# marlam/wurblpt

Measured on AMD Instinct MI355X. Metric: Msamples/s, higher is better.
Workload: dtype f32; 1 GPU; cornell_1024x1024_1024spp_ggx_glass; width=1024, height=1024, spp=1024, triangles=36, bvh_nodes=71, parallelism=1 launch

## Files before the change

wurblpt_amd/csrc/wpt_capi.hip:

```cpp
#include <hip/hip_runtime.h>

#include <algorithm>
#include <atomic>
#include <cassert>
#include <cfloat>
#include <cmath>
#include <cstring>
#include <memory>
#include <string>
#include <vector>

#include "../../include/wurblpt_hip.h"
#include "wpt_pathtrace.inc.h"
#include "wpt_kernel_table.h"
#include "wpt_launch_plan.h"
#include "wpt_scene_layout.h"
#include "wpt_bypass.h"
#include "wpt_wavefront.inc.h"
#include "wpt_postproc.h"
#include "wpt_lightmix.h"
#include "wpt_denoise_launch.h"
#include "wpt_progress.h"
#include "wpt_progress_state.h"

using namespace wptd;
using namespace wptk;

namespace {

__global__ void wpt_selftest_kernel(int op, int n, const float* a, const float* b, float* out)
{
    int i = blockIdx.x * blockDim.x + threadIdx.x;
    if (i >= n)
        return;
    float x = a[i], y = b[i], r;
    switch (op) {
    case 0: r = wptm::sinf_(x); break;
    case 1: r = wptm::cosf_(x); break;
    case 2: r = wptm::expf_(x); break;
    case 3: r = wptm::powf_(x, y); break;
    case 4: r = wptm::asinf_(x); break;
    case 5: r = wptm::atan2f_(x, y); break;
    case 6: r = x / y; break;
    case 7: r = __builtin_sqrtf(x); break;
    case 8: r = x * y + x; break;
    case 10: r = wptm::acosf_(x); break;
    case 11: r = wptm::atan2f_(x, 1.0f); break;
    case 12: r = (float)(2.0 * wptm::asin_d((double)x)); break;
    case 13:
    case 14: {
        float s, c;
        wptm::sincosf_(x, &s, &c);
        r = op == 13 ? s : c;
        break;
    }
    case 15:
    case 16: {
        f2 u;
        u.x = x;
        u.y = y;
        const f2 d = inUnitDisk(u);
        r = op == 15 ? d.x : d.y;
        break;
    }
    default: r = 1.0f / x; break;
    }
    out[i] = r;
}

__global__ void wpt_selftest_aabb_kernel(int n, const float* boxes, const float* rays, int32_t* out)
// ... 133 lines not shown
    wptpp::V3 rgb;
    rgb.x = in[3 * i];
    rgb.y = in[3 * i + 1];
    rgb.z = in[3 * i + 2];
    if (op == 0) {
        uint8_t* o = static_cast<uint8_t*>(out) + 3 * i;
        o[0] = wptpp::toSrgbByte<DevicePow>(rgb.x);
        o[1] = wptpp::toSrgbByte<DevicePow>(rgb.y);
        o[2] = wptpp::toSrgbByte<DevicePow>(rgb.z);
    } else if (op == 3) {
        const float y = wptpp::luminance(rgb);
        if (y > 0.0f)
            atomicMax(maxBits, __float_as_uint(y));
    } else {
        const wptpp::V3 r = op == 1 ? wptpp::uniformRationalQuantization(rgb, a, b) : wptpp::scaleLuminance(rgb, a, b);
        float* o = static_cast<float*>(out) + 3 * i;
        o[0] = r.x;
        o[1] = r.y;
        o[2] = r.z;
    }
}


thread_local std::string g_error;

wpt_status fail(wpt_status s, const std::string& msg)
{
    g_error = msg;
    return s;
}

#define HIP_TRY(expr)                                                                              \
    do {                                                                                           \
        hipError_t e_ = (expr);                                                                    \
        if (e_ != hipSuccess)                                                                      \
            return fail(WPT_ERR_HIP, std::string(#expr) + ": " + hipGetErrorString(e_));           \
    } while (0)
#define WPT_TRY(expr)                                                                              \
    do {                                                                                           \
        const wpt_status s_ = (expr);                                                              \
        if (s_ != WPT_OK)                                                                          \
            return s_;                                                                             \
    } while (0)

}

struct wpt_scene {
    int device;
    SceneView view;
    uint32_t features;
    uint32_t nodeCount, triCount;
    uint32_t foldedLinks;
    uint32_t* ldsLinks = nullptr;
    uint32_t bypassedNodes = 0;
    uint32_t animationCount;
    std::vector<void*> allocations;
    int cuCount;
    std::vector<float> envM, envMcs;
    std::vector<int32_t> envMs;
};

namespace {

uint32_t g_threadsPerGroup = WG;
uint32_t g_variant = 0;
uint32_t g_leaveEighths = 0;
uint32_t g_heavyMin = 0;
uint32_t g_leafBias = 0;
std::atomic<uint32_t> g_lastPasses{1};
std::atomic<const char*> g_kernelName{nullptr};
std::atomic<const char*> g_kernelForm{""};
uint32_t g_topNodes = 65536;
unsigned long long* g_schedStats = nullptr;
uint32_t g_wfMode = 0;
wptk::WfConfig g_wfConfig = { 0, 0, 0, 1, 0, 0, 0, 0, 0 };
uint32_t g_walk = 0;
uint32_t g_bypassMode = wptb::MODE_MODEL;
uint32_t g_slices = 0;
constexpr int SLICE_STATS_DEVICES = 64;
std::atomic<unsigned long long*> g_sliceStats[SLICE_STATS_DEVICES];
std::atomic<unsigned long long*> g_lastSliceStats{nullptr};
static_assert(wptk::PLAN_WG == uint32_t(WG) && wptk::PLAN_SLICE_SLOT_MAX == wptk::SLICE_SLOT_MASK && wptk::SLICE_UNITS_TARGET <= wptk::SLICE_UNITS_MAX
        && wptk::PLAN_FRAME == wptk::SENSOR_FRAME && wptk::PLAN_VIEWS == wptk::SENSOR_VIEWS && wptk::PLAN_ADAPTIVE == wptk::SENSOR_ADAPTIVE
        && wptk::PLAN_SENSORS == wptk::SENSOR_COUNT, "wpt_launch_plan.h restates the kernels' constants and the sensors");
static_assert(wptl::NODE_CHILD == NODE_CHILD && wptl::NODE_INDEX_MASK == NODE_INDEX_MASK && wptl::PRIM_SPHERE == PRIM_SPHERE && wptl::WIDE_STACK == WIDE_STACK
        && wptl::WIDE_NONE == WIDE_NONE && wptl::LDS_SCENE_MAX_BYTES == LDS_SCENE_MAX_BYTES, "wpt_scene_layout.h restates the kernels' node words and limits");

void recordLaunch(const char* name, const char* form, uint32_t passes, unsigned long long* sliceStats)
{
    g_kernelName.store(name, std::memory_order_relaxed);
    g_kernelForm.store(form, std::memory_order_relaxed);
    g_lastPasses.store(passes, std::memory_order_relaxed);
    g_lastSliceStats.store(sliceStats, std::memory_order_relaxed);
}

const char* kernelForm(bool rotated, uint32_t units = 0)
{
    static const std::vector<std::string> forms = [] {
        std::vector<std::string> f;
        for (int r = 0; r < 2; r++)
            for (uint32_t u = 0; u <= wptk::SLICE_UNITS_MAX; u++)
                f.push_back(std::string(r ? "rotated corners" : "") + (u > 1 ? ", sliced x" + std::to_string(u) : std::string()));
        return f;
    }();
    return forms[(rotated ? wptk::SLICE_UNITS_MAX + 1 : 0) + (units <= wptk::SLICE_UNITS_MAX ? units : 0)].c_str();
}

wpt_status lookupKernel(uint32_t features, bool count, bool ldsScene, bool wide, const wptk::KernelEntry** entry)
{
    *entry = wptk::findKernel(features, count, ldsScene, wide);
    if (!*entry)
        return fail(WPT_ERR_UNSUPPORTED, "the library has no kernel wpt_pathtrace<F = " + std::to_string(features) + ", COUNT = " + std::to_string(count)
                + ", LDSSCENE = " + std::to_string(ldsScene) + ", WIDE = " + std::to_string(wide) + ">");
    return WPT_OK;
}

unsigned long long* sliceStatsOfCurrentDevice()
{
    int dev = 0;
    if (hipGetDevice(&dev) != hipSuccess || dev < 0 || dev >= SLICE_STATS_DEVICES)
        return nullptr;
    unsigned long long* p = g_sliceStats[dev].load(std::memory_order_acquire);
    if (!p) {
        if (hipMalloc(reinterpret_cast<void**>(&p), 2 * sizeof(unsigned long long)) != hipSuccess) {
            (void)hipGetLastError();
            return nullptr;
        }
        unsigned long long* expected = nullptr;
        if (!g_sliceStats[dev].compare_exchange_strong(expected, p, std::memory_order_acq_rel)) {
            (void)hipFree(p);
            p = expected;
        }
    }
    return p;
}

template<typename T> wpt_status uploadArray(wpt_scene* s, const T* src, size_t count, const T** dst)
{
    *dst = nullptr;
    size_t bytes = count * sizeof(T);
    void* p = nullptr;
    hipError_t e = hipMalloc(&p, bytes > 0 ? bytes : 16);
    if (e != hipSuccess)
        return fail(e == hipErrorOutOfMemory ? WPT_ERR_OUT_OF_MEMORY : WPT_ERR_HIP, std::string("hipMalloc: ") + hipGetErrorString(e));
    s->allocations.push_back(p);
    if (bytes > 0)
        HIP_TRY(hipMemcpy(p, src, bytes, hipMemcpyHostToDevice));
    *dst = static_cast<const T*>(p);
    return WPT_OK;
}

wpt_status uploadQuads(wpt_scene* s, const std::vector<wptl::Quad>& quads, const float4** dst)
{
    static_assert(sizeof(wptl::Quad) == sizeof(float4), "the layout's quadwords are the device's");
    return uploadArray(s, reinterpret_cast<const float4*>(quads.data()), quads.size(), dst);
}

wpt_status layoutStatus(const wptl::Status& st)
// ... 142 lines not shown
{
    if (!device)
        return fail(WPT_ERR_INVALID_ARGUMENT, "device is NULL");
    HIP_TRY(hipGetDevice(device));
    return WPT_OK;
}

wpt_status wpt_scene_upload(const wpt_scene_desc* desc, wpt_scene** out_scene)
{
    if (!out_scene)
        return fail(WPT_ERR_INVALID_ARGUMENT, "out_scene is NULL");
    *out_scene = nullptr;
    WPT_TRY(validate(desc));
    if (wpt_device_count() <= 0)
        return fail(WPT_ERR_NO_DEVICE, "no HIP device is available; the path tracer has no CPU fallback");
    const uint32_t walk = g_walk, topNodes = g_topNodes;
    std::unique_ptr<wpt_scene, SceneFree> owner(new wpt_scene);
    wpt_scene* s = owner.get();
    SceneView& view = s->view;
    HIP_TRY(hipGetDevice(&s->device));
    s->features = sceneFeatures(desc);
    s->nodeCount = desc->node_count;
    s->triCount = desc->tri_count;
    memset(&view, 0, sizeof(view));
    const std::vector<uint32_t> triNew = wptl::triangleOrder(desc, (walk & WPT_WALK_TRIANGLES_AS_GIVEN) != 0);
    const bool fitsLds = size_t(desc->node_count) * 32 + size_t(desc->tri_count) * 48 <= LDS_SCENE_MAX_BYTES;
    std::vector<uint32_t> ldsNodes;
    {
        wptl::DeviceNodes nodes;
        WPT_TRY(layoutStatus(wptl::deviceNodes(desc, triNew, topNodes, &nodes)));
        view.nodeCount = desc->node_count;
        view.boxesMayBeNan = nodes.boxesMayBeNan;
        WPT_TRY(uploadQuads(s, nodes.quads, &view.nodes));
        s->foldedLinks = 0;
        if (fitsLds) {
            s->foldedLinks = wptl::countFoldedLinks(reinterpret_cast<const uint32_t*>(nodes.quads.data()), desc->node_count, nullptr);
            ldsNodes.resize(size_t(desc->node_count) * 8);
            memcpy(ldsNodes.data(), nodes.quads.data(), ldsNodes.size() * 4);
        }
    }
    if (walk & WPT_WALK_WIDE) {
        const std::vector<wptl::Quad> wide = wptl::wideNodes(desc, triNew);
        if (!wide.empty())
            WPT_TRY(uploadQuads(s, wide, &view.wideNodes));
    }
    {
        const std::vector<wpt_tri_geom> g = wptl::permuted(desc->tri_geom, triNew);
        WPT_TRY(uploadArray(s, reinterpret_cast<const float4*>(g.data()), size_t(desc->tri_count) * 3, &view.triGeom));
        if (fitsLds) {
            const wptb::Plan plan = wptb::plan(ldsNodes.data(), desc->node_count, g.data(), desc->tri_count, g_bypassMode);
            std::vector<uint32_t> words(plan.plain);
            words.insert(words.end(), plan.folded.begin(), plan.folded.end());
            words.insert(words.end(), plan.bypass.begin(), plan.bypass.end());
            const uint32_t* onDevice = nullptr;
            WPT_TRY(uploadArray(s, words.data(), words.size(), &onDevice));
            s->ldsLinks = const_cast<uint32_t*>(onDevice);
            s->bypassedNodes = plan.outCount;
        }
    }
    {
        const std::vector<wpt_tri_attr> a = wptl::permuted(desc->tri_attr, triNew);
        WPT_TRY(uploadArray(s, reinterpret_cast<const float4*>(a.data()), size_t(desc->tri_count) * 6, &view.triAttr));
    }
    WPT_TRY(uploadArray(s, desc->instances, desc->instance_count, &view.instances));
    WPT_TRY(uploadArray(s, desc->materials, desc->material_count, &view.materials));
    view.materialCount = desc->material_count;
    {
        size_t texelCount = 0;
        const std::vector<wpt_texture> devTex = wptl::texelOffsets(desc, &texelCount);
        WPT_TRY(uploadArray(s, devTex.data(), devTex.size(), &view.textures));
        WPT_TRY(decodeTexels(s, desc, devTex, texelCount));
    }
    {
        const std::vector<wpt_hotspot> h = wptl::remappedHotspots(desc, triNew);
        WPT_TRY(uploadArray(s, h.data(), h.size(), &view.hotspots));
    }
    WPT_TRY(uploadArray(s, desc->spheres, desc->sphere_count, &view.spheres));
    WPT_TRY(uploadArray(s, desc->rgl_brdfs, desc->rgl_count, &view.rglBrdfs));
    {
        const wptl::RglPool rgl = wptl::rglPool(desc);
        WPT_TRY(uploadArray(s, rgl.pool.data(), rgl.pool.size(), &view.rglData));
        WPT_TRY(uploadArray(s, rgl.rgbl.data(), rgl.rgbl.size(), &view.rglRgbl));
    }
    WPT_TRY(uploadArray(s, desc->animations, desc->animation_count, &view.animations));
    WPT_TRY(uploadArray(s, desc->keyframes, desc->keyframe_count, &view.keyframes));
    s->animationCount = desc->animation_count;
    view.sphereCount = desc->sphere_count;
    for (int k = 0; k < 6; k++)
        view.envCube[k] = desc->envmap.cube_tex[k];
    {
        hipDeviceProp_t prop;
        s->cuCount = hipGetDeviceProperties(&prop, s->device) == hipSuccess ? prop.multiProcessorCount : 256;
    }
    view.triCount = desc->tri_count;
    view.hotspotCount = desc->hotspot_count;
    view.invHotspotCount = desc->hotspot_count ? 1.0f / float(desc->hotspot_count) : 0.0f;
    if (desc->hotspot_count > 0)
        WPT_TRY(hotspotFaces(s));
    view.envType = desc->envmap.type;
    view.envCompat = desc->envmap.compat;
    view.envTex = desc->envmap.tex;
    view.envN = 0;
    view.envLog2N = -1;
    if (desc->envmap.type != WPT_ENV_NONE && desc->envmap.N > 0) {
        const int N = desc->envmap.N;
        const size_t bins = size_t(N) * N;
// ... 181 lines not shown
    first.carry = second.carry = carry;
    first.cost = cost;
    run(first);
    orderByCost(first, order, work, run.stream, second);
    run(second);
    return true;
}

bool runAdaptiveOrder(const wptk::KernelArgs& args, const SingleKernel& run, StreamScratch& scratch)
{
    uint32_t *cost, *order, *work;
    if (!(cost = scratch.get<uint32_t>(args.blockSize)) || !(order = scratch.get<uint32_t>(args.blockSize)) || !(work = scratch.get<uint32_t>(ORDER_WORK_WORDS)))
        return false;
    wptk::KernelArgs measure = args, ordered = args;
    measure.cost = cost - args.blockStart;
    wptk::launchAdaptiveCost(measure, run.stream);
    orderByCost(measure, order, work, run.stream, ordered);
    run(ordered);
    return true;
}

unsigned long long* runSliced(const wptk::KernelArgs& args, const SingleKernel& runTwin, const wptk::LaunchPlan& plan, StreamScratch& scratch)
{
    unsigned long long* stats = sliceStatsOfCurrentDevice();
    float4* carry;
    uint32_t* words;
    if (!stats || !(carry = scratch.get<float4>(size_t(args.blockSize) * 2)) || !(words = scratch.get<uint32_t>(args.blockSize)))
        return nullptr;
    if (hipMemsetAsync(words, 0, size_t(args.blockSize) * sizeof(uint32_t), runTwin.stream) != hipSuccess
            || hipMemsetAsync(stats, 0, 2 * sizeof(unsigned long long), runTwin.stream) != hipSuccess) {
        (void)hipGetLastError();
        return nullptr;
    }
    wptk::KernelArgs inSlices = args;
    inSlices.slices = { words, carry, stats, plan.rows, plan.units, (g_slices & WPT_SLICES_DECLINE_ODD) ? 1u : 0u };
    runTwin(inSlices);
    return stats;
}

hipError_t runSingleKernel(const wpt_scene* scene, wptk::KernelArgs& args, const wptk::KernelChoice& choice, const wptk::KernelEntry* kernel,
        const wptk::KernelEntry* slicedTwin, const wptk::LaunchPlan& plan, hipStream_t stream)
{
    StreamScratch scratch(stream);
    args.pool = plan.pooled ? scratch.get<uint32_t>(1) : nullptr;
    args.materialsInLds = choice.materialsInLds;
    if (choice.ldsScene) {
        if (!scene->ldsLinks)
            return hipErrorInvalidValue;
        const size_t words = 2 * size_t(scene->nodeCount) + 4;
        const bool fold = (choice.materialsInLds & wptk::LDS_FOLD) != 0;
        const bool bypass = fold && !(g_walk & WPT_WALK_NO_BYPASS) && !args.sv.boxesMayBeNan;
        args.sv.spheres = reinterpret_cast<const wpt_sphere*>(scene->ldsLinks + (fold ? words : 0));
        args.sv.wideNodes = reinterpret_cast<const float4*>(scene->ldsLinks + (bypass ? 2 * words : fold ? words : 0));
    }
    const SingleKernel run = { kernel, dim3((args.blockSize + WG - 1) / WG), choice.sceneLdsBytes, stream };
    bool done = false;
    unsigned long long* sliceStats = nullptr;
    if (args.pool && plan.strategy == wptk::TWO_PASSES)
        done = runTwoPasses(args, run, scratch);
    else if (args.pool && plan.strategy == wptk::ADAPTIVE_ORDER)
        done = runAdaptiveOrder(args, run, scratch);
    else if (args.pool && plan.strategy == wptk::SLICED)
        done = (sliceStats = runSliced(args, SingleKernel{ slicedTwin, run.grid, run.sceneLdsBytes, stream }, plan, scratch)) != nullptr;
    if (!done)
        run(args);
    recordLaunch(kernel->name, kernelForm(choice.rotated, sliceStats ? plan.units : 0), done ? plan.passes : 1u, sliceStats);
    return hipGetLastError();
}

wpt_status renderLaunch(const LaunchRequest& rq)
{
    const bool planes = rq.sensor == wptk::SENSOR_TRANSIENT || rq.sensor == wptk::SENSOR_TOF, views = rq.sensor == wptk::SENSOR_VIEWS;
    if (!rq.scene || !rq.camera || !rq.params || !(rq.frame || planes))
        return fail(WPT_ERR_INVALID_ARGUMENT, "NULL argument");
    const uint32_t cameraCount = views ? rq.views.viewCount : 1u;
    const wpt_status checked = checkFrameBlock(rq.width, rq.height, &rq.samplesSqrt, rq.blockStart, rq.bandStride ? 0u : rq.blockSize, cameraCount);
    if (checked != WPT_OK || rq.blockSize == 0)
        return checked;
    KernelArgs args = {};
    uint32_t need = 0;
    const bool count = rq.counters != nullptr;
    WPT_TRY(launchSetUp(rq.scene, rq.camera, cameraCount, views, rq.params, rq.width, rq.height, rq.samplesSqrt, rq.blockStart,
            rq.blockSize, rq.bandPixels, rq.bandFirst, rq.bandStride, count, args, need));
    args.frame = rq.frame;
    args.counters = rq.counters;
    args.schedStats = g_schedStats;
    if (views)
        args.views = rq.views;
    else if (rq.sensor == wptk::SENSOR_ADAPTIVE)
        args.adaptive = rq.adaptive;
    else if (planes)
        args.bins = rq.bins;
    args.rowStop = rq.samplesSqrt;
    const wptk::KernelChoice choice = wptk::selectKernel({ need, rq.sensor, count, rq.scene->nodeCount, rq.scene->triCount,
            uint32_t(rq.scene->view.materialCount), rq.scene->view.wideNodes != nullptr, g_variant, g_walk });
    const wptk::KernelEntry *kernel = nullptr, *slicedTwin = nullptr;
    wpt_status found = lookupKernel(choice.features, choice.count, choice.ldsScene, choice.wide, &kernel);
    if (found == WPT_OK && choice.sceneInLds && rq.sensor == wptk::SENSOR_FRAME && !count)
        found = lookupKernel(choice.features | FEAT_SLICED, choice.count, choice.ldsScene, choice.wide, &slicedTwin);
    if (found != WPT_OK)
        return found;
    const bool rgl = (need & FEAT_RGL) != 0;
    hipStream_t stream = static_cast<hipStream_t>(rq.stream);
    const wptk::LaunchPlan plan = wptk::planLaunch({ rq.sensor, count, rgl, (need & FEAT_ANIM) != 0, choice.sceneInLds, rq.blockSize, rq.samplesSqrt,
            uint32_t(rq.scene->cuCount), g_variant, g_wfMode, g_slices });
    if (plan.wavefront) {
        uint32_t launches = 0;
        const hipError_t e = wptk::renderWavefront(args, rgl ? wptk::wfFullRgl() : (choice.basic ? wptk::wfBasic() : wptk::wfFull()), g_wfConfig, stream, &launches);
        if (e == hipSuccess) {
            recordLaunch("wf_trace + wf_shade", "", launches, nullptr);
            return WPT_OK;
        }
        if (!plan.wavefrontFallBack || e != hipErrorOutOfMemory)
            return fail(e == hipErrorOutOfMemory ? WPT_ERR_OUT_OF_MEMORY : WPT_ERR_HIP, std::string("wavefront render: ") + hipGetErrorString(e));
        (void)hipGetLastError();
    }
    HIP_TRY(runSingleKernel(rq.scene, args, choice, kernel, slicedTwin, plan, stream));
    return WPT_OK;
}
// ... 1362 lines not shown
```

wurblpt_amd/csrc/wpt_device.h:

```cpp
#ifndef WPT_DEVICE_H
#define WPT_DEVICE_H

#include <hip/hip_runtime.h>
#include <stdint.h>

#include "../../include/wurblpt_hip.h"
#include "wpt_math.h"
#include "wpt_triangle.h"
#include "wpt_anim.h"
#include "wpt_rgl.h"

namespace wptd {

#define WPT_CALL static inline __device__ __attribute__((noinline))


WPT_D float dot(f2 a, f2 b) { float d = 0.0f; d += a.x * b.x; d += a.y * b.y; return d; }
WPT_D float dot(f3 a, f3 b) { float d = 0.0f; d += a.x * b.x; d += a.y * b.y; d += a.z * b.z; return d; }
WPT_D f3 normalize(f3 v) { return divs(v, __builtin_sqrtf(dot(v, v))); }
WPT_D f3 cross(f3 v, f3 w) { return mk3(v.y * w.z - v.z * w.y, v.z * w.x - v.x * w.z, v.x * w.y - v.y * w.x); }
WPT_D f3 reflect(f3 i, f3 n) { return sub(i, scl(2.0f * dot(n, i), n)); }
WPT_D f3 refract(f3 i, f3 n, float eta)
{
    const float d = dot(n, i);
// ... 386 lines not shown
    wptanim::applyTrs(T, sp.center, r.center);
    r.radius = sp.radius * m;
    return r;
}

#ifdef WPT_SPHERE_HIT_INLINE
#define WPT_SPHERE_HIT WPT_D
#else
#define WPT_SPHERE_HIT static __device__ __attribute__((noinline))
#endif
template<uint32_t F = 0> WPT_SPHERE_HIT Hit finishSphereHit(SphereScene sv, Candidate c, f3 org, f3 dir, float time = 0.0f)
{
    wpt_sphere sp = sv.spheres[c.prim & ~PRIM_SPHERE];
    if ((F & FEAT_ANIM) && sp.animation >= 0) {
        const wpt_animation a = sv.animations[sp.animation];
        sp = sphereMoved(sp, wptanim::at<DeviceAnimMath>(sv.keyframes + a.first_keyframe, a.keyframe_count, time));
    }
    Hit h;
    h.a = c.a;
    h.prim = c.prim;
    h.material = sp.material;
    h.p = add(org, scl(c.a, dir));
    f3 n = normalize(sub(h.p, ld3(sp.center)));
    const f3 rn = quatRotate(sp.rotation, n);
    const float alpha = wptm::atan2f_(rn.x, rn.z);
    const float beta = wptm::asinf_(clampr(rn.y, -1.0f, +1.0f));
    h.tc.x = 0.5f * k_inv_pi * (alpha + k_pi);
    h.tc.y = k_inv_pi * (beta + 0.5f * k_pi);
    f3 t = mk3(wptm::cosf_(alpha), 0.0f, -wptm::sinf_(alpha));
    if (__builtin_fabsf(dot(rn, t)) >= k_cosOrthoAngleTolerance)
        t = mk3(0.0f, 0.0f, 0.0f);
    h.backside = false;
    if (dot(n, neg(dir)) < 0.0f) {
        h.backside = true;
        n = neg(n);
    }
    h.n = n;
    h.t = t;
    return h;
}

struct TriGeomFromScene {
    const float4* triGeom;
    WPT_D float4 operator()(uint32_t i) const { return triGeom[i]; }
};
template<uint32_t F = 0, class Tri4 = TriGeomFromScene>
WPT_D Hit finishHit(const SceneView& sv, const Candidate& c, f3 org, f3 dir, float time, Tri4 tri4)
{
    if ((F & FEAT_SPHERES) && (c.prim & PRIM_SPHERE))
        return finishSphereHit<F>(sphereScene(sv), c, org, dir, time);
    Hit h;
    h.a = c.a;
    h.prim = c.prim;
    const float4 g0 = tri4(3 * c.prim + 0);
    const float4 g1 = tri4(3 * c.prim + 1);
    const float4 g2 = tri4(3 * c.prim + 2);
    const uint32_t instance = __float_as_uint(g0.w);
    h.material = __float_as_uint(g1.w);
    const uint32_t flags = __float_as_uint(g2.w);
    const bool backfacing = c.invDet < 0.0f;
    const float bx = c.invDet * c.U, by = c.invDet * c.V, bz = c.invDet * c.W;
    h.p = add(org, scl(c.a, dir));
    const float4* at = sv.triAttr + 6 * (size_t)c.prim;
    const float4 a0 = at[0], a1 = at[1], a2 = at[2], a3 = at[3], a4 = at[4], a5 = at[5];
    const f3 n0 = mk3(a0.x, a0.y, a0.z), n1 = mk3(a0.w, a1.x, a1.y), n2 = mk3(a1.z, a1.w, a2.x);
    f3 nrm = add(add(scl(bx, n0), scl(by, n1)), scl(bz, n2));
    const bool transform = (flags & WPT_TRI_TRANSFORM) != 0;
    const float* N = sv.instances[instance].N;
    if (transform)
        nrm = mat3mul(N, nrm);
    float animationN[9];
    const bool animate = (F & FEAT_ANIM) && (flags & WPT_TRI_ANIMATE);
    if (animate) {
        const wptanim::Trs T = animationAt(sv, sv.instances[instance].animation, time);
        wptanim::toMat3(T.q, animationN);
        nrm = mat3mul(animationN, nrm);
    }
    nrm = normalize(nrm);
    if (backfacing)
        nrm = neg(nrm);
    h.n = nrm;
    h.tc.x = 0.0f;
    h.tc.y = 0.0f;
    if (flags & WPT_TRI_HAVE_TEXCOORDS) {
        h.tc.x = bx * a2.y + by * a2.w + bz * a3.y;
        h.tc.y = bx * a2.z + by * a3.x + bz * a3.z;
    }
    f3 tan = mk3(0.0f, 0.0f, 0.0f);
    if (flags & WPT_TRI_HAVE_TANGENTS) {
        const f3 t0 = mk3(a3.w, a4.x, a4.y), t1 = mk3(a4.z, a4.w, a5.x), t2 = mk3(a5.y, a5.z, a5.w);
        tan = add(add(scl(bx, t0), scl(by, t1)), scl(bz, t2));
        if (dot(tan, tan) > 0.0f) {
            if (transform)
                tan = mat3mul(N, tan);
            if (animate)
                tan = mat3mul(animationN, tan);
            tan = normalize(sub(tan, scl(dot(nrm, tan), nrm)));
        }
    }
    h.t = tan;
    h.backside = backfacing;
    return h;
}
template<uint32_t F = 0>
WPT_D Hit finishHit(const SceneView& sv, const Candidate& c, f3 org, f3 dir, float time = 0.0f)
{
    TriGeomFromScene fromScene;
    fromScene.triGeom = sv.triGeom;
    return finishHit<F>(sv, c, org, dir, time, fromScene);
}

WPT_D float srgbToRgb(float x)
// ... 799 lines not shown
```

wurblpt_amd/csrc/wpt_pathtrace.inc.h:

```cpp
#ifndef WPT_PATHTRACE_INC_H
#define WPT_PATHTRACE_INC_H

#include <hip/hip_runtime.h>

#include "../../include/wurblpt_hip.h"
#include "wpt_blocks.h"

namespace wptk {

using namespace wptd;

constexpr int WG = 256;
constexpr uint32_t NODE_CHILD = 0xc0000000u;
constexpr uint32_t NODE_INDEX_MASK = 0x3fffffffu;
constexpr uint32_t TABLE_BYTES = WPT_MATH_TABLE_WORDS * 8;
constexpr uint32_t COLD_BYTES = TABLE_BYTES + SLOT_COUNT * WG * 16;
constexpr uint32_t LDS_SCENE_MAX_BYTES = 20 * 1024;
constexpr uint32_t LDS_BYTES_PER_WORKGROUP_AT_FOUR = 160 * 1024 / 4;
constexpr uint32_t LDS_MATERIALS = 1u;
constexpr uint32_t LDS_FOLD = 2u;
static_assert(sizeof(wpt_material) % 16 == 0 && alignof(wpt_material) <= 16, "wpt_material must be a whole number of quadwords");
struct ViewsView {
    const wpt_camera* cams;
    uint32_t viewPixels;
    uint32_t viewCount;
};
struct AdaptiveView {
    const uint16_t* samplesSqrt;
    float* moments;
};
struct SlicesView {
    uint32_t* words;
    float4* carry;
    unsigned long long* stats;
    uint32_t rows, units;
    uint32_t declineOdd;
};
constexpr uint32_t SLICE_UNITS_MAX = 15;
constexpr uint32_t SLICE_SLOT_BITS = 28;
constexpr uint32_t SLICE_SLOT_MASK = (1u << SLICE_SLOT_BITS) - 1u;
struct KernelArgs {
    SceneView sv;
    wpt_camera cam;
    wpt_params par;
    uint32_t width, height, samplesSqrt;
    float invWidth, invHeight, invSamplesSqrt, invSamples;
    uint32_t blockStart, blockSize;
    uint32_t tiled;
    uint32_t bandPixels, bandFirst, bandStride;
    uint32_t leaveEighths;
    uint32_t heavyMin;
    uint32_t leafBias;
    uint32_t waitBelow;
    uint32_t fuse;
    uint32_t shadowWalksEnd;
    float* frame;
    uint32_t* pool;
    uint32_t rowStop;
    float4* carry;
    uint32_t* cost;
    const uint32_t* order;
    const uint32_t* orderCount;
    uint32_t cuCount;
    uint32_t materialsInLds;
    wpt_counters* counters;
    unsigned long long* schedStats;
    union {
        BinsView bins;
        ViewsView views;
        AdaptiveView adaptive;
        SlicesView slices;
    };
};
// ... 5 lines not shown
    bool inBlock = gid < args.blockSize;
    if (args.tiled) {
        const uint32_t tilesPerRow = args.width >> 3;
        const uint32_t tile = gid >> 6, lane = gid & 63u;
        const uint32_t tx = tile % tilesPerRow;
        uint32_t ty = tile / tilesPerRow;
        if (args.bandStride) {
            const uint32_t tileRowsPerBand = args.bandPixels / (args.width << 3);
            ty = (args.bandFirst + (ty / tileRowsPerBand) * args.bandStride) * tileRowsPerBand + ty % tileRowsPerBand;
        }
        pixel = args.blockStart + ((ty << 3) + (lane >> 3)) * args.width + (tx << 3) + (lane & 7u);
    } else if (args.bandStride) {
        pixel = (args.bandFirst + (gid / args.bandPixels) * args.bandStride) * args.bandPixels + gid % args.bandPixels;
    } else {
        pixel = args.blockStart + gid;
    }
    if (args.bandStride && pixel >= args.width * args.height)
        inBlock = false;
    if (!inBlock)
        pixel = args.blockStart;
    return inBlock;
}

enum { S_NODE = 0, S_LEAF = 1, S_SHADE = 2, S_NEEEND = 3, S_NEW = 4, S_DONE = 5, S_START = 6  };

constexpr uint32_t WIDE_STACK = 96;
constexpr uint32_t WIDE_NONE = 0xffffffffu;
constexpr int RAY_WALK_BINARY = 0x80;

WPT_D uint2 exactLinks(const SceneView& sv, uint32_t n)
{
    return *reinterpret_cast<const uint2*>(reinterpret_cast<const char*>(sv.spheres) + (n << 3));
}

template<uint32_t F, bool COUNT, bool LDSSCENE, int OCC, bool WIDE = false>
__global__ __launch_bounds__(WG, OCC) void wpt_pathtrace(const KernelArgs args)
{
    static_assert(!WIDE || (!LDSSCENE && !COUNT), "the wide walk: product kernels that fetch the scene from HBM (counting launches walk like the reference)");
    static_assert(!LDSSCENE || !(F & FEAT_SPHERES), "the LDS copy of the tree tells leaves (complemented word) from inner nodes by the sign bit: triangle leaves only");
    static_assert(!((F & FEAT_VIEWS) && (F & FEAT_TRANSIENT)), "a batch of views has no transient film (they share KernelArgs' union)");
    static_assert(!((F & FEAT_ADAPTIVE) && (F & (FEAT_VIEWS | FEAT_TRANSIENT))), "adaptive sampling has no views and no transient film (they share KernelArgs' union)");
    static_assert(!((F & FEAT_ADAPTIVE) && COUNT), "adaptive sampling has no counting build");
    static_assert(!((F & FEAT_TOF) && ((F & (FEAT_VIEWS | FEAT_TRANSIENT | FEAT_ADAPTIVE)) || COUNT)), "the time-of-flight sensor: one view, no other film, no counting build");
    static_assert(!((F & FEAT_SLICED) && ((F & (FEAT_VIEWS | FEAT_TRANSIENT | FEAT_ADAPTIVE | FEAT_TOF)) || COUNT)), "pixels in slices: plain product launches (they share KernelArgs' union)");
    static_assert(!LDSSCENE || (!WIDE && !(F & FEAT_SPHERES)), "the kernels with the scene in LDS carry their link words in SceneView::wideNodes and ::spheres (wpt_device.h): they may read neither as what it is named");
    constexpr bool VIEWS = (F & FEAT_VIEWS) != 0;
    constexpr bool ADAPTIVE = (F & FEAT_ADAPTIVE) != 0;
    constexpr bool SLICED = (F & FEAT_SLICED) != 0;
    constexpr bool ROTATED = (F & FEAT_ROTATED) != 0;
    static_assert(!ROTATED || (LDSSCENE && !(F & FEAT_ANIM)), "rotated copies of the corners: scenes at rest in LDS");
    constexpr bool PREFETCH = !LDSSCENE && !WIDE;
    constexpr int STEPS = LDSSCENE ? 3 : 1;
    constexpr int NEE_IN_WALK = LDSSCENE ? 0 : 4;
    extern __shared__ float4 lds[];
    float4* const ldsCold = lds + TABLE_BYTES / 16;
    float4* const ldsScene = ldsCold + SLOT_COUNT * WG;
#if defined(WPT_MATH_TABLES_IN_LDS) && defined(__HIP_DEVICE_COMPILE__)
    wptm::tables_to_lds(threadIdx.x);
#endif

    SceneView svInLds = args.sv;
    const SceneView& sv = LDSSCENE ? static_cast<const SceneView&>(svInLds) : args.sv;
    const wpt_params& par = args.par;
    const uint32_t nodeCount = sv.nodeCount;

    if (LDSSCENE) {
        const uint32_t n4 = 2 * nodeCount, t4 = 3 * sv.triCount;
        for (uint32_t i = threadIdx.x; i < n4; i += WG) {
            float4 q = sv.nodes[i];
            if (i & 1) {
                const uint2 links = reinterpret_cast<const uint2*>(sv.wideNodes)[i >> 1];
                q.z = __uint_as_float(links.x);
                q.w = __uint_as_float(links.y);
            }
            ldsScene[i] = q;
        }
        if (threadIdx.x < 2)
            ldsScene[n4 + threadIdx.x] = threadIdx.x == 0 ? make_float4(0.0f, 0.0f, 0.0f, 0.0f)
                    : make_float4(0.0f, 0.0f, __uint_as_float(nodeCount), __uint_as_float(nodeCount));
        for (uint32_t i = threadIdx.x; i < t4; i += WG)
            ldsScene[n4 + 2 + i] = sv.triGeom[i];
        if (ROTATED) {
            for (uint32_t i = threadIdx.x; i < t4; i += WG) {
                const float4 g = sv.triGeom[i];
                ldsScene[n4 + 2 + t4 + i] = make_float4(g.y, g.z, g.x, g.w);
                ldsScene[n4 + 2 + 2 * t4 + i] = make_float4(g.z, g.x, g.y, g.w);
            }
        }
        const uint32_t c4 = ROTATED ? 3 * t4 : t4;
        if (args.materialsInLds & LDS_MATERIALS) {
            const uint32_t m4 = sv.materialCount * (uint32_t)(sizeof(wpt_material) / 16);
            const float4* from = reinterpret_cast<const float4*>(sv.materials);
            for (uint32_t i = threadIdx.x; i < m4; i += WG)
                ldsScene[n4 + 2 + c4 + i] = from[i];
            svInLds.materials = reinterpret_cast<const wpt_material*>(ldsScene + n4 + 2 + c4);
        }
    }
    __syncthreads();
    auto node4 = [&](uint32_t i) -> float4 {
        if constexpr (LDSSCENE)
            return ldsScene[i];
        else
            return sv.nodes[i];
    };
    auto tri4 = [&](uint32_t i) -> float4 {
        if constexpr (LDSSCENE)
            return ldsScene[2 * nodeCount + 2 + i];
        else
            return sv.triGeom[i];
    };

    uint32_t walkStart = 0;
    if constexpr (LDSSCENE)
        walkStart = reinterpret_cast<const uint2*>(sv.wideNodes)[nodeCount + 1].x;

    auto pixelOf = [&](uint32_t gid, uint32_t& pixel) -> bool { return lanePixel(args, gid, pixel); };
    const bool firstPass = !ADAPTIVE && args.rowStop < args.samplesSqrt;
    const uint32_t laneLimit = args.order ? *args.orderCount : args.blockSize;
    uint32_t sliceUnits = 1, sliceRows = 0;
    if constexpr (SLICED) {
        sliceUnits = args.pool ? args.slices.units : 1u;
        sliceRows = args.pool ? args.slices.rows : args.samplesSqrt;
    }
    FrameArgs fa;
    fa.cam = args.cam;
    fa.par = args.par;
    fa.width = args.width;
    fa.height = args.height;
    fa.samplesSqrt = args.samplesSqrt;
    fa.invWidth = args.invWidth;
    fa.invHeight = args.invHeight;
    fa.invSamplesSqrt = args.invSamplesSqrt;

    std::conditional_t<ADAPTIVE, PathLdsSum<WG>, PathLds<WG>> ps;
    ps.base = ldsCold + threadIdx.x;
    uint32_t view = 0;
    uint32_t laneSqrt = 0;
    uint32_t unit = 0;
    auto startPixel = [&](uint32_t at) -> bool {
        uint32_t pixel = args.blockStart;
// ... 110 lines not shown
            if (idle != 0) {
                const uint32_t lane = __builtin_amdgcn_mbcnt_hi(~0u, __builtin_amdgcn_mbcnt_lo(~0u, 0u));
                const uint32_t want = (uint32_t)__popcll(idle);
                const int leader = __ffsll((long long)idle) - 1;
                uint32_t first = 0;
                if ((int)lane == leader)
                    first = atomicAdd(args.pool, want);
                first = (uint32_t)__builtin_amdgcn_readlane((int)first, leader);
                if constexpr (SLICED)
                    poolDry = first + want >= sliceUnits * laneLimit;
                else
                    poolDry = first + want >= laneLimit;
                if (state == S_DONE) {
                    const uint32_t rank = __builtin_amdgcn_mbcnt_hi((uint32_t)(idle >> 32), __builtin_amdgcn_mbcnt_lo((uint32_t)idle, 0u));
                    if (startPixel(first + rank))
                        state = S_NEW;
                }
            }
        }
    };

    for (;;) {
        sec<COUNT>(lc, SEC_LOOK);
        const int cTrav = __popcll(__ballot(state == S_NODE || state == S_LEAF));
        const int cShade = __popcll(__ballot(state == S_SHADE));
        const int cNee = __popcll(__ballot(state == S_NEEEND));
        const int cNew = __popcll(__ballot(state == S_NEW));
        if ((cTrav | cShade | cNee | cNew) == 0)
            break;
        int pick;
        const bool fused = args.fuse != 0;
        {
            const int heavyMin = (int)args.heavyMin < 1 ? 1 : (int)args.heavyMin;
            if (fused) {
                pick = (cShade + cNee + cNew >= heavyMin || cTrav == 0) ? (int)S_SHADE : (int)S_NODE;
            } else if (cShade >= heavyMin) {
                pick = S_SHADE;
            } else if (cNee >= heavyMin) {
                pick = S_NEEEND;
            } else if (cNew >= heavyMin) {
                pick = S_NEW;
            } else if (cTrav != 0) {
                pick = S_NODE;
            } else {
                int most = cShade;
                pick = S_SHADE;
                if (cNee > most) { pick = S_NEEEND; most = cNee; }
                if (cNew > most) { pick = S_NEW; most = cNew; }
            }
        }
        long long tBlock = 0;
        if (COUNT)
            tBlock = clock64();
        if (pick == S_NODE) {
            int leaveBelow = (cTrav * (int)args.leaveEighths + 7) >> 3;
            leaveBelow = leaveBelow < 1 ? 1 : leaveBelow;
            if (COUNT)
                sched[0]++;
            float4 pn0 = make_float4(0.0f, 0.0f, 0.0f, 0.0f), pn1 = pn0;
            bool nanPossible = sv.boxesMayBeNan != 0 || __ballot((aux.k & RAY_MAY_NAN) != 0 && (state == S_NODE || state == S_LEAF)) != 0;
                auto binaryStep = [&]() {
                if (COUNT)
                    lc.nodes++;
                const float4 n0 = PREFETCH ? pn0 : node4(2 * node), n1 = PREFETCH ? pn1 : node4(2 * node + 1);
                const uint32_t skip = __float_as_uint(n1.z);
                const uint32_t word = __float_as_uint(n1.w);
                bool hit = boxTest<false>(nodeLo(n0, n1), nodeHi(n0, n1), ps.o, aux.inv, par.min_hit_distance, amax);
                if (nanPossible)
                    hit = boxTest<true>(nodeLo(n0, n1), nodeHi(n0, n1), ps.o, aux.inv, par.min_hit_distance, amax);
                const bool inner = word >= NODE_CHILD;
                const bool toLeaf = hit && !inner;
                leafPrim = toLeaf ? word : leafPrim;
                node = (hit && inner) ? (word & NODE_INDEX_MASK) : skip;
                state = toLeaf ? (int)S_LEAF : (int)S_NODE;
                if (!toLeaf && node >= nodeCount)
                    state = endOfRayState();
                if (PREFETCH && state == S_NODE) {
                    pn0 = node4(2 * node);
                    pn1 = node4(2 * node + 1);
                }
            };
            auto ldsStep = [&](auto nanCheck) {
                const float4 n0 = node4(2 * node), n1 = node4(2 * node + 1);
                uint32_t skip = __float_as_uint(n1.z);
                uint32_t word = __float_as_uint(n1.w);
                if constexpr (decltype(nanCheck)::value) {
                    const uint2 exact = exactLinks(sv, node);
                    skip = exact.x;
                    word = exact.y;
                }
                const bool hit = boxTest<decltype(nanCheck)::value>(nodeLo(n0, n1), nodeHi(n0, n1), ps.o, aux.inv, par.min_hit_distance, amax);
                const bool toLeaf = hit && (int32_t)word < 0;
                leafNode = toLeaf ? node : leafNode;
                state = toLeaf ? (int)S_LEAF : state;
                node = hit ? (toLeaf ? nodeCount : word) : skip;
            };
            if (PREFETCH && state == S_NODE) {
                pn0 = node4(2 * node);
                pn1 = node4(2 * node + 1);
            }
            for (;;) {
                sec<COUNT>(lc, SEC_LOOK_INNER);
                if (LDSSCENE && state == S_NODE && node >= nodeCount)
                    state = endOfRayState();
                const int nNode = __popcll(__ballot(state == S_NODE));
                const int nLeaf = __popcll(__ballot(state == S_LEAF));
                if (nNode + nLeaf < leaveBelow)
                    break;
                if (NEE_IN_WALK > 0 && !COUNT) {
                    const int nNee = __popcll(__ballot(state == S_NEEEND));
                    if (nNee >= NEE_IN_WALK) {
                        if (state == S_NEEEND)
                            afterBlock(blockNeeEnd<F>(sv, par, tri4, ps, best, args.bins));
                        if (state == S_START) {
                            beginRay();
                            if (PREFETCH) {
                                pn0 = node4(2 * node);
                                pn1 = node4(2 * node + 1);
                            }
                        }
                        nanPossible = nanPossible || __ballot((aux.k & RAY_MAY_NAN) != 0 && state == S_NODE) != 0;
                        continue;
                    }
                }
                if (nLeaf * (int)args.leafBias >= nNode * 8 && nLeaf > 0) {
                    if (COUNT) {
                        sched[3]++;
                        sched[4] += nLeaf;
                    }
                    sec<COUNT>(lc, SEC_LEAF_TEST, state == S_LEAF);
                    if (state == S_LEAF) {
                        if (COUNT)
                            lc.leaves++;
                        if constexpr (LDSSCENE) {
                            const float4 n1 = node4(2 * leafNode + 1);
                            leafPrim = ~__float_as_uint(n1.w);
                            node = __float_as_uint(n1.z);
                            if (nanPossible)
                                node = exactLinks(sv, leafNode).x;
                        }
                        Candidate c;
                        bool accepted;
                        if ((F & FEAT_SPHERES) && (leafPrim & PRIM_SPHERE)) {
                            c.invDet = c.U = c.V = c.W = 0.0f;
                            accepted = sphereTest(sphereNow<F>(sv, ps, sv.spheres[leafPrim & ~PRIM_SPHERE]), ps.o, ps.d, par.min_hit_distance, amax, c.a);
                        } else if constexpr (ROTATED) {
                            const uint32_t at = (((uint32_t)aux.k >> 8) & 0x7fffffu) + 3 * leafPrim;
                            const float4 g0 = tri4(at), g1 = tri4(at + 1), g2 = tri4(at + 2);
                            accepted = triangleTestRotated(mk3(g0.x, g0.y, g0.z), mk3(g1.x, g1.y, g1.z), mk3(g2.x, g2.y, g2.z), orgRotated, aux.Sx, aux.Sy,
                                    auxSz, (uint32_t)aux.k & (uint32_t)RAY_FLIP, par.min_hit_distance, amax, c);
                        } else {
                            const float4 g0 = tri4(3 * leafPrim), g1 = tri4(3 * leafPrim + 1), g2 = tri4(3 * leafPrim + 2);
                            f3 v0 = mk3(g0.x, g0.y, g0.z), v1 = mk3(g1.x, g1.y, g1.z), v2 = mk3(g2.x, g2.y, g2.z);
                            if ((F & FEAT_ANIM) && (__float_as_uint(g2.w) & WPT_TRI_ANIMATE)) {
                                const float* animationM = animationMatrix(sv, ps, sv.instances[__float_as_uint(g0.w)].animation);
                                v0 = animatePoint(animationM, v0);
                                v1 = animatePoint(animationM, v1);
                                v2 = animatePoint(animationM, v2);
                            }
                            accepted = triangleTest(v0, v1, v2, ps.o, aux, par.min_hit_distance, amax, c);
                        }
                        const bool grown = WIDE && accepted && !(aux.k & (RAY_MAY_NAN | RAY_WALK_BINARY)) && !(c.a <= amax);
                        if (accepted) {
                            c.prim = leafPrim;
                            best = c;
                            amax = c.a;
                        }
                        if (WIDE && !(aux.k & (RAY_MAY_NAN | RAY_WALK_BINARY)))
                            state = curRef == WIDE_NONE ? endOfRayState() : (int)S_NODE;
                        else
                            state = node >= nodeCount ? endOfRayState() : (int)S_NODE;
                        if ((F & FEAT_ENVMAP) && args.shadowWalksEnd && accepted && ps.rayKind == RAY_NEE_ENV) {
                            state = S_NEEEND;
                            if (LDSSCENE)
                                node = nodeCount;
                        } else if (grown) {
                            aux.k |= RAY_WALK_BINARY;
                            node = 0;
                            amax = k_maxval;
                            best.prim = NO_HIT;
                            state = S_NODE;
                        }
                        if (PREFETCH && state == S_NODE) {
                            pn0 = node4(2 * node);
                            pn1 = node4(2 * node + 1);
                        }
                    }
                } else {
                    if (COUNT) {
                        sched[1]++;
                        sched[2] += nNode;
                    }
                    if constexpr (WIDE) {
                        if (state == S_NODE && !(aux.k & (RAY_MAY_NAN | RAY_WALK_BINARY))) {
                            const uint32_t ref = curRef;
                            const bool admitted = curEntry <= amax;
                            uint2 top = make_uint2(WIDE_NONE, 0u);
                            if (sp > 0)
                                top = pend[sp - 1];
                            curRef = WIDE_NONE;
                            if (admitted && ref < NODE_CHILD) {
                                leafPrim = ref;
// ... 252 lines not shown
```

Before: 1466 Msamples/s.

## Pack leaf links into rotated triangle words and set walk priority

For rotated-corner kernels, leaf node words now encode the node index and the triangle's corner offset, and the triangle w slots in LDS hold the skip and exact links plus the triangle index. A leaf visit then reads its three triangle quadwords and gets the next node from them, with no separate node fetch when the mapping is one-to-one. The change also raises wave priority during the node walk, inserts an explicit waitcnt, and reads hit metadata from global triangle words. The cost is a larger upload with extra leaf-word tables, plus a fallback path for trees that are not one-to-one.

Result: faster. 1495 Msamples/s, median of 6 (+2.0%).

```diff
diff --git a/wurblpt_amd/csrc/wpt_capi.hip b/wurblpt_amd/csrc/wpt_capi.hip
--- a/wurblpt_amd/csrc/wpt_capi.hip
+++ b/wurblpt_amd/csrc/wpt_capi.hip
@@ -16,6 +16,7 @@
 #include "wpt_launch_plan.h"
 #include "wpt_scene_layout.h"
 #include "wpt_bypass.h"
+#include "wpt_leaf_words.h"
 #include "wpt_wavefront.inc.h"
 #include "wpt_postproc.h"
 #include "wpt_lightmix.h"
@@ -255,6 +256,7 @@
     uint32_t nodeCount, triCount;
     uint32_t foldedLinks;
     uint32_t* ldsLinks = nullptr;
+    bool leafOneToOne = false;
     uint32_t bypassedNodes = 0;
     uint32_t animationCount;
     std::vector<void*> allocations;
@@ -289,6 +291,10 @@
 static_assert(wptl::NODE_CHILD == NODE_CHILD && wptl::NODE_INDEX_MASK == NODE_INDEX_MASK && wptl::PRIM_SPHERE == PRIM_SPHERE && wptl::WIDE_STACK == WIDE_STACK
         && wptl::WIDE_NONE == WIDE_NONE && wptl::LDS_SCENE_MAX_BYTES == LDS_SCENE_MAX_BYTES, "wpt_scene_layout.h restates the kernels' node words and limits");
 
+static_assert(wptw::LEAF_NODE_SHIFT == wptk::LEAF_NODE_SHIFT && wptw::LEAF_NODE_MAX == wptk::LEAF_NODE_MAX && wptw::LEAF_CORNER_MASK == wptk::LEAF_CORNER_MASK
+        && LDS_SCENE_MAX_BYTES / 32 <= wptw::LEAF_NODE_MAX && LDS_SCENE_MAX_BYTES / 16 <= wptw::LEAF_CORNER_MASK,
+        "wpt_leaf_words.h restates the rotated kernels' leaf word, which has room for every tree that fits LDS");
+
 void recordLaunch(const char* name, const char* form, uint32_t passes, unsigned long long* sliceStats)
 {
     g_kernelName.store(name, std::memory_order_relaxed);
@@ -297,16 +303,17 @@
     g_lastSliceStats.store(sliceStats, std::memory_order_relaxed);
 }
 
-const char* kernelForm(bool rotated, uint32_t units = 0)
+const char* kernelForm(bool rotated, uint32_t units = 0, bool leafLinksFromNodes = false)
 {
     static const std::vector<std::string> forms = [] {
         std::vector<std::string> f;
-        for (int r = 0; r < 2; r++)
+        for (int r = 0; r < 3; r++)
             for (uint32_t u = 0; u <= wptk::SLICE_UNITS_MAX; u++)
-                f.push_back(std::string(r ? "rotated corners" : "") + (u > 1 ? ", sliced x" + std::to_string(u) : std::string()));
+                f.push_back(std::string(r ? "rotated corners" : "") + (r == 2 ? ", leaf links from the nodes" : "")
+                        + (u > 1 ? ", sliced x" + std::to_string(u) : std::string()));
         return f;
     }();
-    return forms[(rotated ? wptk::SLICE_UNITS_MAX + 1 : 0) + (units <= wptk::SLICE_UNITS_MAX ? units : 0)].c_str();
+    return forms[(rotated ? (leafLinksFromNodes ? 2 : 1) * (wptk::SLICE_UNITS_MAX + 1) : 0) + (units <= wptk::SLICE_UNITS_MAX ? units : 0)].c_str();
 }
 
 wpt_status lookupKernel(uint32_t features, bool count, bool ldsScene, bool wide, const wptk::KernelEntry** entry)
@@ -555,6 +562,14 @@
             std::vector<uint32_t> words(plan.plain);
             words.insert(words.end(), plan.folded.begin(), plan.folded.end());
             words.insert(words.end(), plan.bypass.begin(), plan.bypass.end());
+            s->leafOneToOne = true;
+            for (const std::vector<uint32_t>* links : { &plan.plain, &plan.folded, &plan.bypass }) {
+                const wptw::LeafWords leaf = wptw::leafWords(links->data(), desc->node_count, desc->tri_count);
+                if (leaf.verdict == wptw::TOO_LARGE)
+                    return fail(WPT_ERR_UNSUPPORTED, "a tree that fits LDS has indices beyond its leaf words");
+                s->leafOneToOne = s->leafOneToOne && leaf.verdict == wptw::ONE_TO_ONE;
+                words.insert(words.end(), leaf.words.begin(), leaf.words.end());
+            }
             const uint32_t* onDevice = nullptr;
             WPT_TRY(uploadArray(s, words.data(), words.size(), &onDevice));
             s->ldsLinks = const_cast<uint32_t*>(onDevice);
@@ -842,6 +857,14 @@
         const bool bypass = fold && !(g_walk & WPT_WALK_NO_BYPASS) && !args.sv.boxesMayBeNan;
         args.sv.spheres = reinterpret_cast<const wpt_sphere*>(scene->ldsLinks + (fold ? words : 0));
         args.sv.wideNodes = reinterpret_cast<const float4*>(scene->ldsLinks + (bypass ? 2 * words : fold ? words : 0));
+        if (choice.rotated) {
+            const size_t leafWords = wptw::leafWordsSize(scene->nodeCount, scene->triCount);
+            const uint32_t* sets = scene->ldsLinks + 3 * words;
+            args.sv.spheres = reinterpret_cast<const wpt_sphere*>(sets + (fold ? leafWords : 0));
+            args.sv.wideNodes = reinterpret_cast<const float4*>(sets + (bypass ? 2 * leafWords : fold ? leafWords : 0));
+            if (scene->leafOneToOne)
+                args.materialsInLds |= wptk::LDS_LEAF_LINKS;
+        }
     }
     const SingleKernel run = { kernel, dim3((args.blockSize + WG - 1) / WG), choice.sceneLdsBytes, stream };
     bool done = false;
@@ -854,7 +877,8 @@
         done = (sliceStats = runSliced(args, SingleKernel{ slicedTwin, run.grid, run.sceneLdsBytes, stream }, plan, scratch)) != nullptr;
     if (!done)
         run(args);
-    recordLaunch(kernel->name, kernelForm(choice.rotated, sliceStats ? plan.units : 0), done ? plan.passes : 1u, sliceStats);
+    recordLaunch(kernel->name, kernelForm(choice.rotated, sliceStats ? plan.units : 0, choice.rotated && !scene->leafOneToOne), done ? plan.passes : 1u,
+            sliceStats);
     return hipGetLastError();
 }
 
diff --git a/wurblpt_amd/csrc/wpt_device.h b/wurblpt_amd/csrc/wpt_device.h
--- a/wurblpt_amd/csrc/wpt_device.h
+++ b/wurblpt_amd/csrc/wpt_device.h
@@ -462,12 +462,21 @@
     Hit h;
     h.a = c.a;
     h.prim = c.prim;
-    const float4 g0 = tri4(3 * c.prim + 0);
-    const float4 g1 = tri4(3 * c.prim + 1);
-    const float4 g2 = tri4(3 * c.prim + 2);
-    const uint32_t instance = __float_as_uint(g0.w);
-    h.material = __float_as_uint(g1.w);
-    const uint32_t flags = __float_as_uint(g2.w);
+    uint32_t instance, flags;
+    if constexpr ((F & FEAT_ROTATED) != 0) {
+        (void)tri4;
+        const uint32_t* words = reinterpret_cast<const uint32_t*>(sv.triGeom + 3 * (size_t)c.prim);
+        instance = words[3];
+        h.material = words[7];
+        flags = words[11];
+    } else {
+        const float4 g0 = tri4(3 * c.prim + 0);
+        const float4 g1 = tri4(3 * c.prim + 1);
+        const float4 g2 = tri4(3 * c.prim + 2);
+        instance = __float_as_uint(g0.w);
+        h.material = __float_as_uint(g1.w);
+        flags = __float_as_uint(g2.w);
+    }
     const bool backfacing = c.invDet < 0.0f;
     const float bx = c.invDet * c.U, by = c.invDet * c.V, bz = c.invDet * c.W;
     h.p = add(org, scl(c.a, dir));
diff --git a/wurblpt_amd/csrc/wpt_leaf_words.h b/wurblpt_amd/csrc/wpt_leaf_words.h
--- /dev/null
+++ b/wurblpt_amd/csrc/wpt_leaf_words.h
@@ -0,0 +1,67 @@
+#ifndef WPT_LEAF_WORDS_H
+#define WPT_LEAF_WORDS_H
+
+#include <cstddef>
+#include <cstdint>
+#include <vector>
+
+namespace wptw {
+
+constexpr uint32_t LEAF_BIT = 0x80000000u;
+constexpr uint32_t LEAF_NODE_SHIFT = 16;
+constexpr uint32_t LEAF_NODE_MAX = 0x7fffu;
+constexpr uint32_t LEAF_CORNER_MASK = 0xffffu;
+
+enum Verdict {
+    ONE_TO_ONE = 0,
+    NOT_ONE_TO_ONE = 1,
+    TOO_LARGE = 2
+};
+
+inline uint32_t leafWord(uint32_t node, uint32_t triangle) { return LEAF_BIT | (node << LEAF_NODE_SHIFT) | (3u * triangle); }
+inline uint32_t leafWordNode(uint32_t word) { return (word >> LEAF_NODE_SHIFT) & LEAF_NODE_MAX; }
+inline uint32_t leafWordCorner(uint32_t word) { return word & LEAF_CORNER_MASK; }
+
+inline size_t leafWordsSize(uint32_t nodeCount, uint32_t triCount) { return 2 * size_t(nodeCount) + 4 + ((size_t(triCount) + 1) & ~size_t(1)); }
+inline size_t leafWordsTriangles(uint32_t nodeCount) { return 2 * size_t(nodeCount) + 4; }
+
+struct LeafWords {
+    std::vector<uint32_t> words;
+    Verdict verdict;
+};
+
+inline LeafWords leafWords(const uint32_t* links, uint32_t nodeCount, uint32_t triCount)
+{
+    LeafWords r;
+    r.verdict = ONE_TO_ONE;
+    if (nodeCount > LEAF_NODE_MAX || 3 * uint64_t(triCount) > LEAF_CORNER_MASK) {
+        r.verdict = TOO_LARGE;
+        return r;
+    }
+    const size_t tris = leafWordsTriangles(nodeCount);
+    r.words.assign(links, links + tris);
+    r.words.resize(leafWordsSize(nodeCount, triCount), nodeCount);
+    std::vector<uint32_t> named(triCount, 0u);
+    for (uint32_t i = 0; i < nodeCount; i++) {
+        const uint32_t word = links[2 * size_t(i) + 1];
+        if (!(word & LEAF_BIT))
+            continue;
+        const uint32_t triangle = ~word;
+        if (triangle >= triCount) {
+            r.words[2 * size_t(i) + 1] = leafWord(i, 0u);
+            r.verdict = NOT_ONE_TO_ONE;
+            continue;
+        }
+        r.words[2 * size_t(i) + 1] = leafWord(i, triangle);
+        r.words[tris + triangle] = links[2 * size_t(i)];
+        named[triangle] += 1;
+    }
+    for (uint32_t t = 0; t < triCount; t++)
+        if (named[t] != 1)
+            r.verdict = NOT_ONE_TO_ONE;
+    return r;
+}
+
+}
+
+#endif
diff --git a/wurblpt_amd/csrc/wpt_pathtrace.inc.h b/wurblpt_amd/csrc/wpt_pathtrace.inc.h
--- a/wurblpt_amd/csrc/wpt_pathtrace.inc.h
+++ b/wurblpt_amd/csrc/wpt_pathtrace.inc.h
@@ -19,6 +19,8 @@
 constexpr uint32_t LDS_BYTES_PER_WORKGROUP_AT_FOUR = 160 * 1024 / 4;
 constexpr uint32_t LDS_MATERIALS = 1u;
 constexpr uint32_t LDS_FOLD = 2u;
+constexpr uint32_t LDS_LEAF_LINKS = 4u;
+constexpr uint32_t LEAF_NODE_SHIFT = 16, LEAF_NODE_MAX = 0x7fffu, LEAF_CORNER_MASK = 0xffffu;
 static_assert(sizeof(wpt_material) % 16 == 0 && alignof(wpt_material) <= 16, "wpt_material must be a whole number of quadwords");
 struct ViewsView {
     const wpt_camera* cams;
@@ -130,6 +132,7 @@
     constexpr bool PREFETCH = !LDSSCENE && !WIDE;
     constexpr int STEPS = LDSSCENE ? 3 : 1;
     constexpr int NEE_IN_WALK = LDSSCENE ? 0 : 4;
+    constexpr int PRIORITY_WALK = 2, PRIORITY_LONG = 0;
     extern __shared__ float4 lds[];
     float4* const ldsCold = lds + TABLE_BYTES / 16;
     float4* const ldsScene = ldsCold + SLOT_COUNT * WG;
@@ -156,14 +159,20 @@
         if (threadIdx.x < 2)
             ldsScene[n4 + threadIdx.x] = threadIdx.x == 0 ? make_float4(0.0f, 0.0f, 0.0f, 0.0f)
                     : make_float4(0.0f, 0.0f, __uint_as_float(nodeCount), __uint_as_float(nodeCount));
-        for (uint32_t i = threadIdx.x; i < t4; i += WG)
-            ldsScene[n4 + 2 + i] = sv.triGeom[i];
         if (ROTATED) {
+            const uint32_t* const triSkip = reinterpret_cast<const uint32_t*>(sv.wideNodes) + n4 + 4;
+            const uint32_t* const triExact = reinterpret_cast<const uint32_t*>(sv.spheres) + n4 + 4;
             for (uint32_t i = threadIdx.x; i < t4; i += WG) {
                 const float4 g = sv.triGeom[i];
-                ldsScene[n4 + 2 + t4 + i] = make_float4(g.y, g.z, g.x, g.w);
-                ldsScene[n4 + 2 + 2 * t4 + i] = make_float4(g.z, g.x, g.y, g.w);
-            }
+                const uint32_t tri = i / 3u, corner = i - 3u * tri;
+                const float w = __uint_as_float(corner == 0 ? triSkip[tri] : corner == 1 ? triExact[tri] : tri);
+                ldsScene[n4 + 2 + i] = make_float4(g.x, g.y, g.z, w);
+                ldsScene[n4 + 2 + t4 + i] = make_float4(g.y, g.z, g.x, w);
+                ldsScene[n4 + 2 + 2 * t4 + i] = make_float4(g.z, g.x, g.y, w);
+            }
+        } else {
+            for (uint32_t i = threadIdx.x; i < t4; i += WG)
+                ldsScene[n4 + 2 + i] = sv.triGeom[i];
         }
         const uint32_t c4 = ROTATED ? 3 * t4 : t4;
         if (args.materialsInLds & LDS_MATERIALS) {
@@ -380,6 +389,12 @@
         long long tBlock = 0;
         if (COUNT)
             tBlock = clock64();
+        if constexpr (ROTATED) {
+            if (pick == S_NODE)
+                __builtin_amdgcn_s_setprio(PRIORITY_WALK);
+            else
+                __builtin_amdgcn_s_setprio(PRIORITY_LONG);
+        }
         if (pick == S_NODE) {
             int leaveBelow = (cTrav * (int)args.leaveEighths + 7) >> 3;
             leaveBelow = leaveBelow < 1 ? 1 : leaveBelow;
@@ -419,7 +434,7 @@
                 }
                 const bool hit = boxTest<decltype(nanCheck)::value>(nodeLo(n0, n1), nodeHi(n0, n1), ps.o, aux.inv, par.min_hit_distance, amax);
                 const bool toLeaf = hit && (int32_t)word < 0;
-                leafNode = toLeaf ? node : leafNode;
+                leafNode = toLeaf ? (ROTATED ? word : node) : leafNode;
                 state = toLeaf ? (int)S_LEAF : state;
                 node = hit ? (toLeaf ? nodeCount : word) : skip;
             };
@@ -460,7 +475,20 @@
                     if (state == S_LEAF) {
                         if (COUNT)
                             lc.leaves++;
-                        if constexpr (LDSSCENE) {
+                        float4 r0, r1, r2;
+                        if constexpr (ROTATED) {
+                            const uint32_t at = (((uint32_t)aux.k >> 8) & 0x7fffffu) + (leafNode & LEAF_CORNER_MASK);
+                            __builtin_amdgcn_s_waitcnt(0xc07f);
+                            r0 = tri4(at);
+                            r1 = tri4(at + 1);
+                            r2 = tri4(at + 2);
+                            leafPrim = __float_as_uint(r2.w);
+                            node = __float_as_uint(nanPossible ? r1.w : r0.w);
+                            if (!(args.materialsInLds & LDS_LEAF_LINKS)) {
+                                const uint32_t leaf = (leafNode >> LEAF_NODE_SHIFT) & LEAF_NODE_MAX;
+                                node = nanPossible ? exactLinks(sv, leaf).x : __float_as_uint(node4(2 * leaf + 1).z);
+                            }
+                        } else if constexpr (LDSSCENE) {
                             const float4 n1 = node4(2 * leafNode + 1);
                             leafPrim = ~__float_as_uint(n1.w);
                             node = __float_as_uint(n1.z);
@@ -473,9 +501,7 @@
                             c.invDet = c.U = c.V = c.W = 0.0f;
                             accepted = sphereTest(sphereNow<F>(sv, ps, sv.spheres[leafPrim & ~PRIM_SPHERE]), ps.o, ps.d, par.min_hit_distance, amax, c.a);
                         } else if constexpr (ROTATED) {
-                            const uint32_t at = (((uint32_t)aux.k >> 8) & 0x7fffffu) + 3 * leafPrim;
-                            const float4 g0 = tri4(at), g1 = tri4(at + 1), g2 = tri4(at + 2);
-                            accepted = triangleTestRotated(mk3(g0.x, g0.y, g0.z), mk3(g1.x, g1.y, g1.z), mk3(g2.x, g2.y, g2.z), orgRotated, aux.Sx, aux.Sy,
+                            accepted = triangleTestRotated(mk3(r0.x, r0.y, r0.z), mk3(r1.x, r1.y, r1.z), mk3(r2.x, r2.y, r2.z), orgRotated, aux.Sx, aux.Sy,
                                     auxSz, (uint32_t)aux.k & (uint32_t)RAY_FLIP, par.min_hit_distance, amax, c);
                         } else {
                             const float4 g0 = tri4(3 * leafPrim), g1 = tri4(3 * leafPrim + 1), g2 = tri4(3 * leafPrim + 2);
```
